# kei312/stereoanywhere

Hardware: AMD Instinct MI355X
Metric: stereo pairs/sec @540x960 D=192 (1/2/4/8 GPU) + EPE vs reference (higher is better)
Workload: dtype f32 (F(4x4) Winograd-domain and direct-conv products as exact f16 hi/lo pair products on MFMA, fp32 accumulation; everything else fp32); 1 GPU; configs[1]: batch 4/GPU x 540x960 (padded 544x960), 22 GRU iters, published flags; global_batch=4, iters=22, parallelism=dp1 (independent pairs, metrics all_gather)

## Files before the change

stereoanywhere_amd/csrc/conv2d_wino4.hip:

```cpp
#include "sa_common.h"

#include <algorithm>
#include <cstdlib>
#include <type_traits>

#pragma clang fp contract(fast)

namespace {

using sa::f32x4, sa::f32x2, sa::f16x2, sa::f16x4;

constexpr int NPT = 36;

template <int NW_, int KC_, bool SPLIT_ = false>
struct W4Cfg {
  static constexpr bool SPLIT = SPLIT_;
  static constexpr int NW = NW_, NTHR = 64 * NW_, TG = NW_ / 2, NT = 16 * TG, KC = KC_, JPC = KC_ / 4;
  static constexpr int NR = 6;
  static constexpr int CO = 32, CG = 2;
  static constexpr int SB = 4 * CO;
  static constexpr int PS_MAX = NT == 64 ? 340 : 204;
  static constexpr int PBUF = (KC * PS_MAX + 63) / 64 * 64 * 4;
  static constexpr int UBUF = NPT * KC * CO;
  static constexpr int BUF = PBUF + UBUF;
// ... 526 lines not shown
    __syncthreads();
  }
#pragma unroll 1
  for (int kc = 0; kc < nchunks; ++kc) {
    const int cur = kc & 1;
    if constexpr (AFF) {
      asm volatile("s_waitcnt vmcnt(0)" ::: "memory");
      float *pbuf = smem + cur * BUF;
#pragma unroll
      for (int j = 0; j < PDMA; ++j) {
        const int pcj = (int)((pcs >> (4 * j)) & 15u) - 1;
        if (pcj >= 0) {
          f32x4 *q = reinterpret_cast<f32x4 *>(pbuf + ((wv + NWAVE * j) * 64 + lane) * 4);
          const float2 ab = atab[kc * KC + pcj];
          f32x4 v = *q;
#pragma unroll
          for (int e = 0; e < 4; ++e) v[e] = fmaxf(v[e] * ab.x + ab.y, act_floor);
          *q = v;
        }
      }
    }
    if constexpr (SPLIT && !AFF) {
      if (scaled) {
        asm volatile("s_waitcnt vmcnt(0)" ::: "memory");
        float *pbuf = smem + cur * BUF + (wv * 64 + lane) * 4;
#pragma unroll 1
        for (int j = 0; j < PDMA; ++j) {
          if (wv + NWAVE * j < npi) {
            f32x4 *q = reinterpret_cast<f32x4 *>(pbuf + NWAVE * j * 256);
            *q = *q * xscale;
          }
        }
      }
    }
    __syncthreads();
    const float *pb = smem + cur * BUF + pread;
    const float *ub = smem + cur * BUF + PBUF + uread;
    f32x2 ra[6], rc[6];
    f32x4 rb[6];
    auto load_rows = [&](int s, int r0, int r1) __attribute__((always_inline)) {
      const float *p = pb + s * 4 * PSv * 4;
#pragma unroll
      for (int r = r0; r < r1; ++r) {
        ra[r] = *reinterpret_cast<const f32x2 *>(p + r * PGv * 4);
        rb[r] = *reinterpret_cast<const f32x4 *>(p + r * PGv * 4 + 2);
        rc[r] = *reinterpret_cast<const f32x2 *>(p + r * PGv * 4 + 6);
      }
    };
    f32xg bc[NR], bn[NR];
    auto load_b = [&](int s, int jj, f32xg *b) __attribute__((always_inline)) {
#pragma unroll
      for (int i = 0; i < NR; ++i) {
        if constexpr (SPLIT) {
          const float *q = ub + (6 * i + 3 * HF + jj) * JPC * SB + s;
          b[i] = f32xg{q[0], q[JPC]};
        } else {
          b[i] = *reinterpret_cast<const f32xg *>(ub + ((6 * i + 3 * HF + jj) * JPC + s) * SB);
        }
      }
    };
    if constexpr (W4Paired<C, AFF>) {
      float t0[6][3], t1[6][3];
      load_rows(0, 0, 6);
#pragma unroll
      for (int r = 0; r < 6; ++r) bt6h<HF>(ra[r].y, rb[r].x, rb[r].y, rb[r].z, rb[r].w, rc[r].x, t0[r]);
      load_rows(1, 0, 6);
#pragma unroll
      for (int r = 0; r < 6; ++r) bt6h<HF>(ra[r].y, rb[r].x, rb[r].y, rb[r].z, rb[r].w, rc[r].x, t1[r]);
      f32x4 pc_[NR];
      auto load_bp = [&](int jj, int i0, int i1, f32x4 (&b)[NR]) __attribute__((always_inline)) {
#pragma unroll
        for (int i = i0; i < i1; ++i) b[i] = *reinterpret_cast<const f32x4 *>(ub + (6 * i + 3 * HF + jj) * JPC * SB);
      };
#pragma unroll
      for (int jj = 0; jj < 3; ++jj) {
        if (kc + 1 < nchunks) {
          issue_part(kc + 1, cur ^ 1, jj);
          __builtin_amdgcn_sched_barrier(0);
        }
        load_bp(jj, 0, NR / 2, pc_);
        float v0[6], v1[6];
        bt6(t0[0][jj], t0[1][jj], t0[2][jj], t0[3][jj], t0[4][jj], t0[5][jj], v0);
        bt6(t1[0][jj], t1[1][jj], t1[2][jj], t1[3][jj], t1[4][jj], t1[5][jj], v1);
#pragma unroll
        for (int i = 0; i < NR; ++i) {
          if (i == 1) load_bp(jj, NR / 2, NR, pc_);
          if constexpr (HALF) {
            const f16x4 ahi = w4_pair_half(v0[i], v1[i]);
#pragma unroll
            for (int g = 0; g < CG; ++g) {
              const f16x4 bp = __builtin_bit_cast(f16x4, g == 0 ? pc_[i].xy : pc_[i].zw);
              acc[i][jj][g] = __builtin_amdgcn_mfma_f32_16x16x16f16(ahi, bp, acc[i][jj][g], 0, 0, 0);
            }
          } else {
            f16x4 ahi, alo;
            w4_pair_split(v0[i], v1[i], ahi, alo);
#pragma unroll
            for (int g = 0; g < CG; ++g) {
              const f16x4 bp = __builtin_bit_cast(f16x4, g == 0 ? pc_[i].xy : pc_[i].zw);
              acc[i][jj][g] = __builtin_amdgcn_mfma_f32_16x16x16f16(ahi, bp, acc[i][jj][g], 0, 0, 0);
              acc[i][jj][g] = __builtin_amdgcn_mfma_f32_16x16x16f16(alo, bp, acc[i][jj][g], 0, 0, 0);
            }
          }
        }
        __builtin_amdgcn_sched_barrier(0);
      }
    } else {
      load_rows(0, 0, 6);
      load_b(0, 0, bc);
#pragma unroll
      for (int s = 0; s < JPC; ++s) {
        if (s == 1) load_rows(1, 3, 6);
        float t[6][3];
#pragma unroll
        for (int r = 0; r < 6; ++r) bt6h<HF>(ra[r].y, rb[r].x, rb[r].y, rb[r].z, rb[r].w, rc[r].x, t[r]);
        if (s + 1 < JPC) load_rows(1, 0, 3);
#pragma unroll
        for (int jj = 0; jj < 3; ++jj) {
          if (s == 0 && kc + 1 < nchunks) {
            issue_part(kc + 1, cur ^ 1, jj);
            __builtin_amdgcn_sched_barrier(0);
          }
          if (s + 1 < JPC || jj < 2) load_b(jj < 2 ? s : s + 1, jj < 2 ? jj + 1 : 0, bn);
          float v[6];
          bt6(t[0][jj], t[1][jj], t[2][jj], t[3][jj], t[4][jj], t[5][jj], v);
          if constexpr (SPLIT) {
            static_assert(HALF, "an unpaired split config is the half config");
#pragma unroll
            for (int i = 0; i < NR; ++i) {
              const f16x4 a = __builtin_shufflevector(__builtin_convertvector(f32x2{v[i], v[i]}, f16x2),
                                                      f16x2{(_Float16)0.0f, (_Float16)0.0f}, 0, 1, 2, 3);
              const f16x4 b0 = __builtin_bit_cast(f16x4, f32x2{bc[i][0], bc[i][0]});
              const f16x4 b1 = __builtin_bit_cast(f16x4, f32x2{bc[i][1], bc[i][1]});
              acc[i][jj][0] = __builtin_amdgcn_mfma_f32_16x16x16f16(a, b0, acc[i][jj][0], 0, 0, 0);
              acc[i][jj][1] = __builtin_amdgcn_mfma_f32_16x16x16f16(a, b1, acc[i][jj][1], 0, 0, 0);
            }
          } else {
#pragma unroll
            for (int i = 0; i < NR; ++i)
#pragma unroll
              for (int g = 0; g < CG; ++g)
                acc[i][jj][g] = __builtin_amdgcn_mfma_f32_16x16x4f32(v[i], bc[i][g],
                                                                      acc[i][jj][g], 0, 0, 0);
          }
          __builtin_amdgcn_sched_barrier(0);

#pragma unroll
          for (int i = 0; i < NR; ++i) bc[i] = bn[i];
        }
      }
    }
  }
  __syncthreads();
  if constexpr (SPLIT) {
    const float inv_scale = 1.0f / ((float)(1 << W4S_LOG2) * xscale);
#pragma unroll
    for (int i = 0; i < NR; ++i)
#pragma unroll
      for (int jj = 0; jj < 3; ++jj)
#pragma unroll
        for (int g = 0; g < CG; ++g) acc[i][jj][g] *= inv_scale;
  }

  float *ot = smem;
  const int relu = P.relu;
  f32x4 chk = f32x4{0.f, 0.f, 0.f, 0.f};
  float whead = 0.0f;
  if constexpr (GATED && C::NTHR == 512)
    if (gate->mode == 3 && tid < C::CO * 9) whead = gate->head_w[co0 * 9 + tid];
#pragma unroll
  for (int phase = 0; phase < 2; ++phase) {
#pragma unroll
  for (int gi = 0; gi < CG / 2; ++gi) {
    const int g = 2 * gi + (phase == 0 ? 1 - HF : HF);
    const int col = g * 16 + (lane & 15);
    const float bv = phase == 1 ? bpre[gi] : 0.0f;
#pragma unroll
    for (int i = 0; i < 4; ++i) {
      const int ti = tg * 16 + w4_tile_of_row(4 * (lane >> 4) + i), orow = (ti >> ltw) * 4, ocol = (ti & (tw - 1)) * 4;
      float u[4][3];
#pragma unroll
      for (int jj = 0; jj < 3; ++jj) {
        float mcol[6], o[4];
#pragma unroll
        for (int a = 0; a < 6; ++a) mcol[a] = acc[a][jj][g][i];
        at6(mcol, o);
#pragma unroll
        for (int a = 0; a < 4; ++a) u[a][jj] = o[a];
      }
#pragma unroll
      for (int a = 0; a < 4; ++a) {
        const f32x4 y = at6h<HF>(u[a][0], u[a][1], u[a][2]);
        f32x4 *o = reinterpret_cast<f32x4 *>(ot + col * OPP + (orow + a) * BW + ocol);
        if (phase == 0) {
          *o = y;
        } else {
          f32x4 v = (HF == 0 ? (*o + y) : (y + *o)) + bv;
          if constexpr (SPLIT) chk += v;
          if (relu) v = f32x4{fmaxf(v.x, 0.0f), fmaxf(v.y, 0.0f), fmaxf(v.z, 0.0f), fmaxf(v.w, 0.0f)};
          *o = v;
        }
      }
    }
  }
    if (phase == 0) __syncthreads();
  }
  if constexpr (SPLIT) {
    static_assert(C::CO * C::OPP + C::CO * 9 + NWAVE <= C::SMEM, "range guard flags");
    int *flags = reinterpret_cast<int *>(smem + C::CO * C::OPP + C::CO * 9);
    const float t = (chk.x + chk.y) + (chk.z + chk.w);
    const bool wbad = __builtin_amdgcn_ballot_w64(!__builtin_isfinite(t)) != 0;
    if (lane == 0) flags[wv] = wbad ? 1 : 0;
    __syncthreads();
    int any = 0;
#pragma unroll
    for (int w = 0; w < NWAVE; ++w) any |= flags[w];
    if (any && guard) return true;
  } else {
    __syncthreads();
  }
  if constexpr (GATED && C::NTHR == 512) {
    if (gate->mode == 3) {
      w4_flowhead<C, LTW>(P, *gate, smem, n, co0, st, y0, x0, tid, whead);
      return false;
    }
  }
  w4_emit<C, GATED, C::CO>(P, gate, ot, 0, n, co0, st, tiles_w, y0, x0, BH, BW, ltw + 2, tid);
  return false;
}

template <class C, bool GATED, bool AFF = false>
__global__ __launch_bounds__(C::NTHR, C::NW == 8 ? 1 : 2) void wino_f4k3_kernel(const W4Launch L) {
  const unsigned g = blockIdx.x;
  int pi = 0;
#pragma unroll
  for (int i = 1; i < MAX_PROB; ++i) pi += (i < L.nprob && g >= L.end[i - 1]) ? 1 : 0;
  const unsigned base = pi ? L.end[pi - 1] : 0u, nb = L.nblk[pi];
  if (g - base >= nb) return;
  __shared__ __attribute__((aligned(16))) float smem[C::SMEM];
  __shared__ float2 atab[AFF ? C::AFF_MAX : 1];
  const unsigned wid = sa::xcd_remap(g - base, nb);
  const bool guard = C::SPLIT && L.guard;
  const W4Prob &P = L.p[pi];
  const W4Gate *gp = GATED ? &L.gate[pi] : nullptr;
  bool over;
#define W4_BODY(CC_, HF_, LTW_, G_, XS_) w4_body<CC_, HF_, LTW_, GATED, AFF>(P, gp, wid, smem, atab, G_, XS_)
  if (threadIdx.x < C::NTHR / 2) over = P.ltw == 4 ? W4_BODY(C, 0, 4, guard, 1.0f) : W4_BODY(C, 0, 5, guard, 1.0f);
  else over = P.ltw == 4 ? W4_BODY(C, 1, 4, guard, 1.0f) : W4_BODY(C, 1, 5, guard, 1.0f);
  if constexpr (C::SPLIT) {
    if (over) {
      __syncthreads();
      if (threadIdx.x == 0) atomicAdd(&g_w4_redo_blocks, 1u);
      int pil = __builtin_amdgcn_readfirstlane(pi);
      unsigned widl = __builtin_amdgcn_readfirstlane(wid);
      asm volatile("" : "+s"(pil), "+s"(widl));
      const W4Prob &P2 = L.p[pil];
      const W4Gate *gp2 = GATED ? &L.gate[pil] : nullptr;
#define W4_BODY2(HF_, LTW_) w4_body<C, HF_, LTW_, GATED, AFF>(P2, gp2, widl, smem, atab, false, 0.0f)
      if (threadIdx.x < C::NTHR / 2) {
        if (P2.ltw == 4) W4_BODY2(0, 4);
        else W4_BODY2(0, 5);
      } else {
        if (P2.ltw == 4) W4_BODY2(1, 4);
        else W4_BODY2(1, 5);
      }
#undef W4_BODY2
    }
  }
#undef W4_BODY
}

__global__ __launch_bounds__(256) void wino4_weights_kernel(const float *__restrict__ w, int Cout, int Cin, int CB,
                                                            float *__restrict__ U) {
  const long i = (long)blockIdx.x * blockDim.x + threadIdx.x;
  if (i >= (long)Cout * Cin) return;
  const int co = (int)(i / Cin), ci = (int)(i % Cin);
  const float *g = w + i * 9;
  const double G[6][3] = {{0.25, 0.0, 0.0},
                          {-1.0 / 6, -1.0 / 6, -1.0 / 6},
                          {-1.0 / 6, 1.0 / 6, -1.0 / 6},
                          {1.0 / 24, 1.0 / 12, 1.0 / 6},
                          {1.0 / 24, -1.0 / 12, 1.0 / 6},
                          {0.0, 0.0, 1.0}};
  double t[6][3];
  for (int a = 0; a < 6; ++a)
    for (int c = 0; c < 3; ++c) t[a][c] = G[a][0] * g[c] + G[a][1] * g[3 + c] + G[a][2] * g[6 + c];
  const int chunk = ci / 8, s = (ci % 8) / 4, k = ci % 4, cb = co / CB, c = co % CB, ng = CB / 16;
  for (int a = 0; a < 6; ++a)
    for (int b = 0; b < 6; ++b) {
      const double u = t[a][0] * G[b][0] + t[a][1] * G[b][1] + t[a][2] * G[b][2];
      const int pt = 6 * a + b;
      U[(((((long)cb * (Cin / 8) + chunk) * NPT + pt) * 2 + s) * 4 + k) * CB + (c & 15) * ng + (c >> 4)] = (float)u;
    }
}

__global__ __launch_bounds__(256) void wino4s_weights_kernel(const float *__restrict__ w, int Cout, int Cin,
                                                             unsigned *__restrict__ U) {
  const long i = (long)blockIdx.x * blockDim.x + threadIdx.x;
  if (i >= (long)Cout * Cin) return;
  const int co = (int)(i / Cin), ci = (int)(i % Cin);
  const float *g = w + i * 9;
  const double G[6][3] = {{0.25, 0.0, 0.0},
                          {-1.0 / 6, -1.0 / 6, -1.0 / 6},
                          {-1.0 / 6, 1.0 / 6, -1.0 / 6},
                          {1.0 / 24, 1.0 / 12, 1.0 / 6},
                          {1.0 / 24, -1.0 / 12, 1.0 / 6},
                          {0.0, 0.0, 1.0}};
  double t[6][3];
  for (int a = 0; a < 6; ++a)
    for (int c = 0; c < 3; ++c) t[a][c] = G[a][0] * g[c] + G[a][1] * g[3 + c] + G[a][2] * g[6 + c];
  const int chunk = ci / 8, s = (ci % 8) / 4, k = ci % 4, cb = co / 32, gg = (co % 32) / 16, n = co % 16;
  for (int a = 0; a < 6; ++a)
    for (int b = 0; b < 6; ++b) {
      const double u = (t[a][0] * G[b][0] + t[a][1] * G[b][1] + t[a][2] * G[b][2]) * (double)(1 << W4S_LOG2);
      const _Float16 hi = (_Float16)(float)u;
      const _Float16 lo = (_Float16)(float)(u - (double)hi);
      const unsigned pr = (unsigned)__builtin_bit_cast(unsigned short, hi) |
                          ((unsigned)__builtin_bit_cast(unsigned short, lo) << 16);
      const int pt = 6 * a + b;
      U[((((((long)cb * (Cin / 8) + chunk) * NPT + pt) * 4 + k) * 16 + n) * 2 + gg) * 2 + s] = pr;
    }
}


__global__ __launch_bounds__(256) void flow_head_reduce_kernel(const float *__restrict__ part, long part_bs, int ncb,
                                                               int H, int W, int BH, int BW, int tiles_w,
                                                               int tiles_hw, const float *__restrict__ bias0,
                                                               float *__restrict__ cx, float *__restrict__ fa,
                                                               long fa_bs, float *__restrict__ fb, long fb_bs) {
  const unsigned r = blockIdx.x * 256u + threadIdx.x;
  const unsigned hw = (unsigned)(H * W);
  if (r >= hw) return;
  const long b = blockIdx.y;
  const int y = (int)(r / (unsigned)W), x = (int)(r % (unsigned)W);
  const int RH = BH + 2, RW = BW + 2, tiles_h = tiles_hw / tiles_w;
  const int ty0 = y / BH, tx0 = x / BW;
  const bool up = y % BH == 0 && ty0 > 0, dn = y % BH == BH - 1 && ty0 + 1 < tiles_h;
  const bool lf = x % BW == 0 && tx0 > 0, rt = x % BW == BW - 1 && tx0 + 1 < tiles_w;
  const int ty1 = up ? ty0 - 1 : ty0 + 1, tx1 = lf ? tx0 - 1 : tx0 + 1;
  auto off = [&](int ty, int tx) { return ((long)(ty * tiles_w + tx) * RH + (y - (ty * BH - 1))) * RW + (x - (tx * BW - 1)); };
  const bool hy = up || dn, hx = lf || rt;
  const long o0 = off(ty0, tx0), o1 = hx ? off(ty0, tx1) : o0, o2 = hy ? off(ty1, tx0) : o0,
             o3 = hx && hy ? off(ty1, tx1) : o0;
  float d = bias0[0];
  const float *pc = part + b * part_bs;
  const long cbs = (long)tiles_hw * RH * RW;
  for (int cb0 = 0; cb0 < ncb; cb0 += 8) {
    float a[8][4];
#pragma unroll
    for (int j = 0; j < 8; ++j) {
// ... 219 lines not shown
```

stereoanywhere_amd/csrc/conv_direct.hip:

```cpp
#include "sa_common.h"

#pragma clang fp contract(fast)

namespace {

using sa::f32x4, sa::f32x2, sa::f16x2, sa::f16x4;

constexpr float DSP_SCALE = 4096.0f;
__device__ __forceinline__ f16x4 dsplit(const float x) {
  const f16x2 hh = __builtin_convertvector(f32x2{x, x}, f16x2);
  float l;
  asm("v_fma_mix_f32 %0, -%1, 1.0, %2 op_sel_hi:[1,0,0]" : "=v"(l) : "v"(__builtin_bit_cast(unsigned, hh)), "v"(x));
  const f16x2 ll = __builtin_convertvector(f32x2{l, l}, f16x2);
  return __builtin_shufflevector(hh, ll, 0, 1, 2, 3);
}

__device__ __forceinline__ float dunsplit(const float packed) {
  const f16x2 p = __builtin_bit_cast(f16x2, packed);
  return (float)p[0] + (float)p[1];
}

__device__ unsigned g_direct_redo_blocks;

constexpr int DOTH = 8, DOTW = 32, MT = 2;

template <int K, int S, int KC, int NTL, bool DS>
struct DCfg {
  static constexpr int PH = (DOTH - 1) * S + K, PW = (DOTW - 1) * S + K;
  static constexpr int PWP = PW;
  static constexpr int PL0 = PH * PWP, PR = S == 1 ? 16 : 17;
  static constexpr int PLANE = PL0 + ((PR - PL0 % 32) + 32) % 32;
  static constexpr int XN = KC * PLANE;
  static constexpr int NC = 16 * NTL;
  static constexpr int KK = K * K;
  static constexpr int WN = KC * KK * NC;
  static constexpr int DN = DS ? KC * NC : 0;
  static constexpr int NCP = NC + 16;
  static constexpr int WROWS = KC * KK + (DS ? KC : 0);
  static constexpr int XPT = (XN + 511) / 512, WPT = (WN + DN) / 4 / 512 + (((WN + DN) / 4) % 512 ? 1 : 0);
  static constexpr int KSTEPS = KC * KK / 4;
  static constexpr int NACC = NTL * (DS ? 2 : 1);
  static constexpr int SMEM = XN + WROWS * NCP + 4;
  static_assert(KC % 4 == 0, "a K-step of 4 must stay inside one tap");
  static_assert((WN + DN) % 4 == 0, "weights are staged as float4");
  static_assert(SMEM * 4 <= 160 * 1024, "LDS budget");
  static_assert(8 * 2 * NACC * 16 * 2 <= SMEM, "the stats reduction reuses the staging LDS");
};

struct DirArgs {
  const float *in;
  long in_bs;
  const float *skip, *cm, *cs;
  long skip_bs;
  int Cin, H, W, Ho, Wo;
  const float *wg, *wd;
  int Cout, co_blocks, tiles_w, tiles, nchunks;
  float *out, *out_ds;
  long out_bs, out_ds_bs;
  double *part, *part_ds;
};

__device__ __forceinline__ float close_value(float v, float m, float s, float k) {
#pragma clang fp contract(off)
  const float y = fmaxf((v - m) * s + 0.0f, 0.0f);
  return fmaxf(y + k, 0.0f);
}

template <int K, int S, int KC, int NTL, bool DS, bool SP = false, bool CL = false>
__global__ __launch_bounds__(512, DS ? 2 : 4) void conv_direct_kernel(const DirArgs a) {
  using C = DCfg<K, S, KC, NTL, DS>;
  constexpr int NC = C::NC, NCP = C::NCP, PLANE = C::PLANE, PWP = C::PWP;
  __shared__ __attribute__((aligned(16))) float sm[C::SMEM];
  __shared__ float ctab[CL ? 2 : 1][CL ? 2 * KC : 1];
  float *sx = sm, *sw = sm + C::XN, *sd = sw + KC * C::KK * NCP;
  constexpr int SPARE = C::SMEM - 4;
  const int tid = threadIdx.x, lane = tid & 63;
  const int wv = __builtin_amdgcn_readfirstlane(tid >> 6);
  const unsigned wid = sa::xcd_remap(blockIdx.x, gridDim.x);
  const int cb = wid % a.co_blocks;
  const int st = (wid / a.co_blocks) % a.tiles;
  const int n = wid / (a.co_blocks * a.tiles);
  const int oy0 = (st / a.tiles_w) * DOTH, ox0 = (st % a.tiles_w) * DOTW;
  const int iy0 = oy0 * S - K / 2, ix0 = ox0 * S - K / 2;
  const long hw = (long)a.H * a.W;
  const float *src = a.in + (long)n * a.in_bs;

  constexpr int OOB = 0x7ffffff0;
  const __amdgpu_buffer_rsrc_t xin = __builtin_amdgcn_make_buffer_rsrc(
      const_cast<float *>(src), (short)0, (int)((long)a.Cin * hw * 4), 0x00020000);
  int xoff[C::XPT], xl[C::XPT];
#pragma unroll
  for (int j = 0; j < C::XPT; ++j) {
    const int i = tid + 512 * j;
    const int ci = i / PLANE, rem = i % PLANE, r = rem / PWP, c = rem % PWP;
    const int y = iy0 + r, x = ix0 + c;
    const bool ok = i < C::XN && rem < C::PH * PWP && c < C::PW && y >= 0 && y < a.H && x >= 0 && x < a.W;
    xoff[j] = ok ? (int)((min(ci, a.Cin - 1) * hw + (long)y * a.W + x) * 4) : OOB;
    xl[j] = i < C::XN ? i : SPARE;
  }
  constexpr int WQ = (C::WN + C::DN) / 4;
  const __amdgpu_buffer_rsrc_t win = __builtin_amdgcn_make_buffer_rsrc(
      const_cast<float *>(a.wg) + (long)cb * a.nchunks * C::WN, (short)0, (int)((long)a.nchunks * C::WN * 4),
      0x00020000);
  const __amdgpu_buffer_rsrc_t din = __builtin_amdgcn_make_buffer_rsrc(
      const_cast<float *>(DS ? a.wd + (long)cb * a.nchunks * C::DN : a.wg), (short)0,
      (int)((long)a.nchunks * (DS ? C::DN : 0) * 4), 0x00020000);
  int woff[C::WPT], wl[C::WPT];
  bool wds[C::WPT];
#pragma unroll
  for (int j = 0; j < C::WPT; ++j) {
    const int i = tid + 512 * j;
    wds[j] = i >= C::WN / 4;
    woff[j] = i < WQ ? (wds[j] ? (i - C::WN / 4) * 16 : i * 16) : OOB;
    const int row = (4 * i) / NC, col = (4 * i) % NC;
    wl[j] = i < WQ ? row * NCP + col : SPARE;
  }
  const __amdgpu_buffer_rsrc_t kin = __builtin_amdgcn_make_buffer_rsrc(
      const_cast<float *>(CL ? a.skip + (long)n * a.skip_bs : src), (short)0, (int)((long)a.Cin * hw * 4), 0x00020000);
  float xr[C::XPT], kr[CL ? C::XPT : 1];
  float tv = 0.0f;
  f32x4 wr[C::WPT];
  auto fetch = [&](int chunk) __attribute__((always_inline)) {
    const int xs = chunk * KC * (int)hw * 4;
#pragma unroll
    for (int j = 0; j < C::XPT; ++j) xr[j] = __uint_as_float(__builtin_amdgcn_raw_buffer_load_b32(xin, xoff[j], xs, 0));
    if constexpr (CL) {
#pragma unroll
      for (int j = 0; j < C::XPT; ++j) kr[j] = __uint_as_float(__builtin_amdgcn_raw_buffer_load_b32(kin, xoff[j], xs, 0));
      if (tid < 2 * KC) {
        const int c = min(chunk * KC + tid % KC, a.Cin - 1);
        tv = (tid < KC ? a.cm : a.cs)[(long)n * a.Cin + c];
      }
    }
#pragma unroll
    for (int j = 0; j < C::WPT; ++j) {
      const auto v = wds[j] ? __builtin_amdgcn_raw_buffer_load_b128(din, woff[j], chunk * C::DN * 4, 0)
                            : __builtin_amdgcn_raw_buffer_load_b128(win, woff[j], chunk * C::WN * 4, 0);
      wr[j] = f32x4{__uint_as_float(v[0]), __uint_as_float(v[1]), __uint_as_float(v[2]), __uint_as_float(v[3])};
    }
  };
  auto put_tab = [&](int chunk) __attribute__((always_inline)) {
    if (CL && tid < 2 * KC) ctab[CL ? chunk & 1 : 0][tid] = tv;
  };
  auto commit = [&](int chunk) __attribute__((always_inline)) {
#pragma unroll
    for (int j = 0; j < C::XPT; ++j) {
      float v = xr[j];
      if constexpr (CL) {
        const int cl = min((tid + 512 * j) / PLANE, KC - 1);
        const float *tb = ctab[chunk & 1];
        v = xoff[j] == OOB ? 0.0f : close_value(v, tb[cl], tb[KC + cl], kr[j]);
      }
      sx[xl[j]] = v;
    }
#pragma unroll
    for (int j = 0; j < C::WPT; ++j) *reinterpret_cast<f32x4 *>(sw + wl[j]) = wr[j];
  };

  f32x4 acc[MT][C::NACC];
#pragma unroll
  for (int m = 0; m < MT; ++m)
#pragma unroll
    for (int t = 0; t < C::NACC; ++t) acc[m][t] = f32x4{0.f, 0.f, 0.f, 0.f};
  const int kq = lane >> 4, ml = lane & 15;
  int abase[MT];
#pragma unroll
  for (int m = 0; m < MT; ++m) abase[m] = kq * PLANE + (wv * S) * PWP + (m * 16 + ml) * S;
  const int bbase = kq * NCP + ml;

  fetch(0);
  if constexpr (CL) {
    put_tab(0);
    __syncthreads();
  }
  commit(0);
  __syncthreads();
#pragma unroll 1
  for (int chunk = 0; chunk < a.nchunks; ++chunk) {
    if (chunk + 1 < a.nchunks) fetch(chunk + 1);
#pragma unroll
    for (int s = 0; s < C::KSTEPS; ++s) {
      const int tap = (4 * s) / KC, ci0 = (4 * s) % KC;
      const int koff = ci0 * PLANE + (tap / K) * PWP + (tap % K);
      float av[MT];
#pragma unroll
      for (int m = 0; m < MT; ++m) av[m] = sx[abase[m] + koff];
      auto prod = [&](const float bv, f32x4 *ac) __attribute__((always_inline)) {
        if constexpr (SP) {
          const f16x4 b = __builtin_bit_cast(f16x4, f32x2{bv, bv});
#pragma unroll
          for (int m = 0; m < MT; ++m) ac[m * C::NACC] = __builtin_amdgcn_mfma_f32_16x16x16f16(dsplit(av[m]), b, ac[m * C::NACC], 0, 0, 0);
        } else {
#pragma unroll
          for (int m = 0; m < MT; ++m) ac[m * C::NACC] = __builtin_amdgcn_mfma_f32_16x16x4f32(av[m], bv, ac[m * C::NACC], 0, 0, 0);
        }
      };
#pragma unroll
      for (int t = 0; t < NTL; ++t) prod(sw[bbase + 4 * s * NCP + t * 16], &acc[0][t]);
      if (DS && tap == (K / 2) * K + K / 2) {
#pragma unroll
        for (int t = 0; t < NTL; ++t) prod(sd[bbase + ci0 * NCP + t * 16], &acc[0][NTL + t]);
      }
    }
    if (CL && chunk + 1 < a.nchunks) put_tab(chunk + 1);
    __syncthreads();
    if (chunk + 1 < a.nchunks) {
      commit(chunk + 1);
      __syncthreads();
    }
  }
  if constexpr (SP) {
    f32x4 sum = f32x4{0.f, 0.f, 0.f, 0.f};
#pragma unroll
    for (int m = 0; m < MT; ++m)
#pragma unroll
      for (int t = 0; t < C::NACC; ++t) sum += acc[m][t];
    const float tot = (sum.x + sum.y) + (sum.z + sum.w);
    if (__syncthreads_or(!__builtin_isfinite(tot))) {
      if (tid == 0) atomicAdd(&g_direct_redo_blocks, 1u);
#pragma unroll
      for (int m = 0; m < MT; ++m)
#pragma unroll
        for (int t = 0; t < C::NACC; ++t) acc[m][t] = f32x4{0.f, 0.f, 0.f, 0.f};
#pragma unroll 1
      for (int chunk = 0; chunk < a.nchunks; ++chunk) {
        fetch(chunk);
        if constexpr (CL) {
          put_tab(chunk);
          __syncthreads();
        }
        commit(chunk);
        __syncthreads();
#pragma unroll 1
        for (int s = 0; s < C::KSTEPS; ++s) {
          const int tap = (4 * s) / KC, ci0 = (4 * s) % KC;
          const int koff = ci0 * PLANE + (tap / K) * PWP + (tap % K);
#pragma unroll
          for (int t = 0; t < NTL; ++t) {
            const float w = dunsplit(sw[bbase + 4 * s * NCP + t * 16]);
#pragma unroll
            for (int m = 0; m < MT; ++m)
              acc[m][t] = __builtin_amdgcn_mfma_f32_16x16x4f32(sx[abase[m] + koff], w, acc[m][t], 0, 0, 0);
          }
          if (DS && tap == (K / 2) * K + K / 2) {
#pragma unroll
            for (int t = 0; t < NTL; ++t) {
              const float w = dunsplit(sd[bbase + ci0 * NCP + t * 16]);
#pragma unroll
              for (int m = 0; m < MT; ++m)
                acc[m][NTL + t] = __builtin_amdgcn_mfma_f32_16x16x4f32(sx[abase[m] + koff], w, acc[m][NTL + t], 0, 0, 0);
            }
          }
        }
        __syncthreads();
      }
    }
  }

  if constexpr (SP) {
#pragma unroll
    for (int m = 0; m < MT; ++m)
#pragma unroll
      for (int t = 0; t < C::NACC; ++t) acc[m][t] *= 1.0f / DSP_SCALE;
  }
  double *red = reinterpret_cast<double *>(sm);
  constexpr int RC = C::NACC * 16;
  const int oy = oy0 + wv;
  const bool stats = a.part != nullptr;
  const bool interior = oy0 + DOTH <= a.Ho && ox0 + DOTW <= a.Wo && (a.Wo & 3) == 0;
#pragma unroll
  for (int t = 0; t < C::NACC; ++t) {
    const bool ds = DS && t >= NTL;
    const int co = cb * NC + (ds ? t - NTL : t) * 16 + ml;
    float *dst = (ds ? a.out_ds + (long)n * a.out_ds_bs : a.out + (long)n * a.out_bs) + (long)co * a.Ho * a.Wo;
    double s1 = 0.0, s2 = 0.0;
    if (interior) {
#pragma unroll
      for (int m = 0; m < MT; ++m) {
        const int ox = ox0 + m * 16 + 4 * kq;
        *reinterpret_cast<float4 *>(dst + (long)oy * a.Wo + ox) =
            make_float4(acc[m][t][0], acc[m][t][1], acc[m][t][2], acc[m][t][3]);
#pragma unroll
        for (int r = 0; r < 4; ++r) {
          const double v = acc[m][t][r];
          s1 += v;
          s2 += v * v;
        }
      }
    } else {
#pragma unroll
      for (int m = 0; m < MT; ++m) {
        const int ox = ox0 + m * 16 + 4 * kq;
#pragma unroll
        for (int r = 0; r < 4; ++r) {
          if (oy < a.Ho && ox + r < a.Wo) {
            const float v = acc[m][t][r];
            dst[(long)oy * a.Wo + ox + r] = v;
            s1 += (double)v;
            s2 += (double)v * v;
          }
        }
      }
    }
    if (stats) {
      s1 += __shfl_xor(s1, 16);
      s2 += __shfl_xor(s2, 16);
      s1 += __shfl_xor(s1, 32);
      s2 += __shfl_xor(s2, 32);
      if (kq == 0) {
        red[(wv * 2 + 0) * RC + t * 16 + ml] = s1;
        red[(wv * 2 + 1) * RC + t * 16 + ml] = s2;
      }
    }
  }
  if (stats) {
    __syncthreads();
    for (int c = tid; c < RC; c += 512) {
      double s1 = 0.0, s2 = 0.0;
#pragma unroll
      for (int w = 0; w < 8; ++w) {
        s1 += red[(w * 2 + 0) * RC + c];
        s2 += red[(w * 2 + 1) * RC + c];
      }
      const bool ds = DS && c >= NC;
      double *pp = ds ? a.part_ds : a.part;
      if (pp) {
        const int co = cb * NC + (ds ? c - NC : c);
        pp += (((long)n * a.Cout + co) * a.tiles + st) * 2;
        pp[0] = s1;
        pp[1] = s2;
      }
    }
  }
}

__global__ void direct_weights_kernel(const float *__restrict__ w, int Cout, int Cin, int K, int KC, int NC,
                                      int nchunks, int ds, float *__restrict__ out) {
  const long total = (long)Cout * nchunks * KC * K * K;
  const long i = (long)blockIdx.x * blockDim.x + threadIdx.x;
  if (i >= total) return;
  const int n = (int)(i % NC);
  long r = i / NC;
  const int ci = (int)(r % KC);
  r /= KC;
  const int tap = (int)(r % (K * K));
  r /= K * K;
  const int chunk = (int)(r % nchunks);
  const int cblk = (int)(r / nchunks);
  const int co = cblk * NC + n, cin = chunk * KC + ci;
  (void)ds;
  out[i] = cin < Cin ? w[((long)co * Cin + cin) * K * K + tap] : 0.0f;
}

bool pick(int K, int S, int Cout, int &KC, int &NTL) {
  KC = K == 7 ? 4 : 8;
  if (K == 7 && S == 1 && Cout % 64 == 0) { NTL = 4; return true; }
  if ((K == 3 || K == 1) && S == 2 && Cout == 96) { NTL = 6; return true; }
  if ((K == 3 || K == 1) && S == 2 && Cout % 128 == 0) { NTL = 8; return true; }
  return false;
}

}

extern "C" int sa_conv_direct_weights(const float *weight, int Cout, int Cin, int K, int S, int with_ds,
                                      float *out, void *stream) {
  int KC = 0, NTL = 0;
  SA_REQUIRE(weight && out && Cout > 0 && Cin > 0, "sa_conv_direct_weights: bad arguments");
  SA_REQUIRE(pick(K, S, Cout, KC, NTL) && (K != 1 || with_ds), "sa_conv_direct_weights: no kernel for K=%d S=%d Cout=%d",
             K, S, Cout);
  const int NC = 16 * NTL, nchunks = (Cin + KC - 1) / KC;
  const long total = (long)Cout * nchunks * KC * K * K;
  hipStream_t s = sa::as_stream(stream);
  direct_weights_kernel<<<(unsigned)((total + 255) / 256), 256, 0, s>>>(weight, Cout, Cin, K, KC, NC, nchunks, 0,
                                                                       out);
  return sa::check_launch("sa_conv_direct_weights");
}

namespace {
__global__ void direct_split_kernel(const float *__restrict__ w, long n, unsigned *__restrict__ out) {
  const long i = (long)blockIdx.x * blockDim.x + threadIdx.x;
  if (i >= n) return;
  const double u = (double)w[i] * DSP_SCALE;
  const _Float16 hi = (_Float16)(float)u;
  const _Float16 lo = (_Float16)(float)(u - (double)hi);
  out[i] = (unsigned)__builtin_bit_cast(unsigned short, hi) | ((unsigned)__builtin_bit_cast(unsigned short, lo) << 16);
}

}

extern "C" int sa_conv_direct_weights_split(const float *arranged, long n, void *out, void *stream) {
  SA_REQUIRE(arranged && out && n > 0, "sa_conv_direct_weights_split: bad arguments");
  hipStream_t s = sa::as_stream(stream);
  direct_split_kernel<<<(unsigned)((n + 255) / 256), 256, 0, s>>>(arranged, n, static_cast<unsigned *>(out));
  return sa::check_launch("sa_conv_direct_weights_split");
}

long sa_direct_redo_blocks_internal(int reset) {
  return sa::read_redo_counter(g_direct_redo_blocks, reset, false);
}

extern "C" long sa_conv_direct_weights_size(int Cout, int Cin, int K, int S, int with_ds) {
  int KC = 0, NTL = 0;
  if (!pick(K, S, Cout, KC, NTL) || (K == 1 && !with_ds)) return -1;
  return (long)Cout * ((Cin + KC - 1) / KC) * KC * K * K;
}

extern "C" long sa_conv_direct_stat_parts(int Ho, int Wo) {
  return (long)((Wo + DOTW - 1) / DOTW) * ((Ho + DOTH - 1) / DOTH);
}

template <bool SP>
static int conv_direct_launch(const float *in, long in_bs, int N, int Cin, int H, int W, int K, int S,
                              const float *wg, const float *wd, int Cout, float *out, long out_bs, float *out_ds,
                              long out_ds_bs, double *part, double *part_ds, void *stream,
                              const float *skip = nullptr, long skip_bs = 0, const float *cm = nullptr,
                              const float *cs = nullptr) {
  int KC = 0, NTL = 0;
  const bool ds = wd != nullptr, cl = skip != nullptr;
  SA_REQUIRE(in && wg && out && N > 0 && Cin > 0 && H > 0 && W > 0, "sa_conv_direct: bad arguments");
  SA_REQUIRE(!ds || out_ds, "sa_conv_direct: downsample weights without an output");
  SA_REQUIRE(K != 1 && pick(K, S, Cout, KC, NTL) && ds == (S == 2),
             "sa_conv_direct: no kernel for K=%d S=%d Cout=%d ds=%d", K, S, Cout, (int)ds);
  SA_REQUIRE((long)Cin * H * W < (1L << 31), "sa_conv_direct: image too large");
  SA_REQUIRE(Cin % KC == 0 || Cin <= KC, "sa_conv_direct: Cin must be a multiple of %d (or at most %d)", KC, KC);
  SA_REQUIRE(!cl || (cm && cs && K == 3 && Cin % KC == 0),
             "sa_conv_direct_close: needs mean / rstd, a 3x3 stride-2 conv and Cin %% %d == 0", KC);
  const int p = K / 2;
  const int Ho = (H + 2 * p - K) / S + 1, Wo = (W + 2 * p - K) / S + 1;
  const int tiles_w = (Wo + DOTW - 1) / DOTW, tiles = tiles_w * ((Ho + DOTH - 1) / DOTH);
  const int co_blocks = Cout / (16 * NTL);
  const DirArgs a{in, in_bs, skip, cm, cs, skip_bs, Cin, H, W, Ho, Wo, wg, wd, Cout, co_blocks, tiles_w, tiles,
                  (Cin + KC - 1) / KC, out, out_ds, out_bs, out_ds_bs, part, part_ds};
  const long nblk = (long)N * tiles * co_blocks;
  SA_REQUIRE(nblk < (1L << 31), "sa_conv_direct: grid too large");
  hipStream_t s = sa::as_stream(stream);
  sa::TimingScope ts(SA_K_CONV_DIRECT, s);
  if (K == 7) {
    conv_direct_kernel<7, 1, 4, 4, false, SP><<<(unsigned)nblk, 512, 0, s>>>(a);
  } else if (NTL == 6) {
    if (cl) conv_direct_kernel<3, 2, 8, 6, true, SP, true><<<(unsigned)nblk, 512, 0, s>>>(a);
    else conv_direct_kernel<3, 2, 8, 6, true, SP><<<(unsigned)nblk, 512, 0, s>>>(a);
  } else {
    SA_REQUIRE(!cl, "sa_conv_direct_close: no close form for Cout = %d", Cout);
    conv_direct_kernel<3, 2, 8, 8, true, SP><<<(unsigned)nblk, 512, 0, s>>>(a);
  }
  return sa::check_launch("sa_conv_direct");
}

extern "C" int sa_conv_direct(const float *in, long in_bs, int N, int Cin, int H, int W, int K, int S,
                              const float *wg, const float *wd, int Cout, float *out, long out_bs, float *out_ds,
                              long out_ds_bs, double *part, double *part_ds, void *stream) {
  return conv_direct_launch<false>(in, in_bs, N, Cin, H, W, K, S, wg, wd, Cout, out, out_bs, out_ds, out_ds_bs, part,
                                   part_ds, stream);
}

extern "C" int sa_conv_direct_split(const float *in, long in_bs, int N, int Cin, int H, int W, int K, int S,
                                    const void *wg, const void *wd, int Cout, float *out, long out_bs, float *out_ds,
                                    long out_ds_bs, double *part, double *part_ds, void *stream) {
  return conv_direct_launch<true>(in, in_bs, N, Cin, H, W, K, S, static_cast<const float *>(wg),
                                  static_cast<const float *>(wd), Cout, out, out_bs, out_ds, out_ds_bs, part, part_ds,
                                  stream);
}

extern "C" int sa_conv_direct_close_supported(int K, int S, int Cout) {
  int KC = 0, NTL = 0;
  return K == 3 && S == 2 && pick(K, S, Cout, KC, NTL) && NTL == 6 ? 1 : 0;
}

extern "C" int sa_conv_direct_close(const float *c2, long c2_bs, const float *skip, long skip_bs, const float *mean,
                                    const float *rstd, int N, int Cin, int H, int W, int K, int S, const void *wg,
                                    const void *wd, int split, int Cout, float *out, long out_bs, float *out_ds,
                                    long out_ds_bs, double *part, double *part_ds, void *stream) {
  SA_REQUIRE(skip, "sa_conv_direct_close: null skip");
  if (split)
    return conv_direct_launch<true>(c2, c2_bs, N, Cin, H, W, K, S, static_cast<const float *>(wg),
                                    static_cast<const float *>(wd), Cout, out, out_bs, out_ds, out_ds_bs, part, part_ds,
                                    stream, skip, skip_bs, mean, rstd);
  return conv_direct_launch<false>(c2, c2_bs, N, Cin, H, W, K, S, static_cast<const float *>(wg),
                                   static_cast<const float *>(wd), Cout, out, out_bs, out_ds, out_ds_bs, part, part_ds,
                                   stream, skip, skip_bs, mean, rstd);
}
```

Measured before the change: 69.76 pairs/s.

## Pack split-f16 direct-conv operands for 16x16x32 MFMA and fold Winograd rescale into bias

In the split-precision direct conv, weights are pre-split into f16 hi/lo fragments laid out in LDS by tap step. Activations are split eight at a time, so each product runs as three 16x16x32 f16 MFMAs (hi*hi, hi*lo, lo*hi) instead of many 16x16x16 MFMAs with a duplicated operand. The 7x7 stem is limited to a single channel chunk. Separately, the Winograd split path drops the per-accumulator rescale loop and applies the scale with an FMA alongside the bias in the epilogue. This adds a new fragment-staging scheme, more LDS use, and a dropped lo*lo term that the old path may have partly covered.

Measured after the change: 69.95 pairs/s (median of 6 runs). No clear change (+0.3%).

```diff
diff --git a/stereoanywhere_amd/csrc/conv2d_wino4.hip b/stereoanywhere_amd/csrc/conv2d_wino4.hip
--- a/stereoanywhere_amd/csrc/conv2d_wino4.hip
+++ b/stereoanywhere_amd/csrc/conv2d_wino4.hip
@@ -702,15 +702,7 @@
     }
   }
   __syncthreads();
-  if constexpr (SPLIT) {
-    const float inv_scale = 1.0f / ((float)(1 << W4S_LOG2) * xscale);
-#pragma unroll
-    for (int i = 0; i < NR; ++i)
-#pragma unroll
-      for (int jj = 0; jj < 3; ++jj)
-#pragma unroll
-        for (int g = 0; g < CG; ++g) acc[i][jj][g] *= inv_scale;
-  }
+  const float inv_scale = SPLIT ? 1.0f / ((float)(1 << W4S_LOG2) * xscale) : 1.0f;
 
   float *ot = smem;
   const int relu = P.relu;
@@ -745,7 +737,13 @@
         if (phase == 0) {
           *o = y;
         } else {
-          f32x4 v = (HF == 0 ? (*o + y) : (y + *o)) + bv;
+          f32x4 v = HF == 0 ? (*o + y) : (y + *o);
+          if constexpr (SPLIT) {
+            v = f32x4{__builtin_fmaf(v.x, inv_scale, bv), __builtin_fmaf(v.y, inv_scale, bv),
+                      __builtin_fmaf(v.z, inv_scale, bv), __builtin_fmaf(v.w, inv_scale, bv)};
+          } else {
+            v = v + bv;
+          }
           if constexpr (SPLIT) chk += v;
           if (relu) v = f32x4{fmaxf(v.x, 0.0f), fmaxf(v.y, 0.0f), fmaxf(v.z, 0.0f), fmaxf(v.w, 0.0f)};
           *o = v;
diff --git a/stereoanywhere_amd/csrc/conv_direct.hip b/stereoanywhere_amd/csrc/conv_direct.hip
--- a/stereoanywhere_amd/csrc/conv_direct.hip
+++ b/stereoanywhere_amd/csrc/conv_direct.hip
@@ -4,20 +4,26 @@
 
 namespace {
 
-using sa::f32x4, sa::f32x2, sa::f16x2, sa::f16x4;
+using sa::f32x4, sa::f32x2, sa::f16x2, sa::f16x8;
+using u32x4 = __attribute__((ext_vector_type(4))) unsigned;
+using u32x2 = __attribute__((ext_vector_type(2))) unsigned;
 
 constexpr float DSP_SCALE = 4096.0f;
-__device__ __forceinline__ f16x4 dsplit(const float x) {
-  const f16x2 hh = __builtin_convertvector(f32x2{x, x}, f16x2);
-  float l;
-  asm("v_fma_mix_f32 %0, -%1, 1.0, %2 op_sel_hi:[1,0,0]" : "=v"(l) : "v"(__builtin_bit_cast(unsigned, hh)), "v"(x));
-  const f16x2 ll = __builtin_convertvector(f32x2{l, l}, f16x2);
-  return __builtin_shufflevector(hh, ll, 0, 1, 2, 3);
-}
-
-__device__ __forceinline__ float dunsplit(const float packed) {
-  const f16x2 p = __builtin_bit_cast(f16x2, packed);
-  return (float)p[0] + (float)p[1];
+__device__ __forceinline__ void dsplit8(const float (&x)[8], f16x8 &ahi, f16x8 &alo) {
+  f16x2 h[4], q[4];
+#pragma unroll
+  for (int p = 0; p < 4; ++p) {
+    h[p] = __builtin_convertvector(f32x2{x[2 * p], x[2 * p + 1]}, f16x2);
+    float l0, l1;
+    asm("v_fma_mix_f32 %0, -%1, 1.0, %2 op_sel_hi:[1,0,0]" : "=v"(l0) : "v"(__builtin_bit_cast(unsigned, h[p])), "v"(x[2 * p]));
+    asm("v_fma_mix_f32 %0, -%1, 1.0, %2 op_sel:[1,0,0] op_sel_hi:[1,0,0]"
+        : "=v"(l1) : "v"(__builtin_bit_cast(unsigned, h[p])), "v"(x[2 * p + 1]));
+    q[p] = __builtin_convertvector(f32x2{l0, l1}, f16x2);
+  }
+  ahi = __builtin_shufflevector(__builtin_shufflevector(h[0], h[1], 0, 1, 2, 3),
+                                __builtin_shufflevector(h[2], h[3], 0, 1, 2, 3), 0, 1, 2, 3, 4, 5, 6, 7);
+  alo = __builtin_shufflevector(__builtin_shufflevector(q[0], q[1], 0, 1, 2, 3),
+                                __builtin_shufflevector(q[2], q[3], 0, 1, 2, 3), 0, 1, 2, 3, 4, 5, 6, 7);
 }
 
 __device__ unsigned g_direct_redo_blocks;
@@ -41,6 +47,18 @@
   static constexpr int KSTEPS = KC * KK / 4;
   static constexpr int NACC = NTL * (DS ? 2 : 1);
   static constexpr int SMEM = XN + WROWS * NCP + 4;
+  static constexpr int CPL = KC / 4, TPS = 8 / CPL;
+  static constexpr int STEPS = (KK + TPS - 1) / TPS;
+  static constexpr int CT = (K / 2) * K + K / 2;
+  static constexpr int NF = STEPS + (DS ? 1 : 0);
+  static constexpr int FRAG = NTL * 512;
+  static constexpr int PJ = NTL * 64 * 2 <= 512 ? 4 : 8;
+  static constexpr int UPF = NTL * 64 * (8 / PJ);
+  static constexpr int SMEM_SP = XN + NF * FRAG + 4;
+  static_assert(KC == 4 || KC == 8, "a lane holds 1 or 2 channels of a tap");
+  static_assert(!DS || CT % TPS == 0, "the 1x1 takes the first slot of the centre tap's step");
+  static_assert(UPF <= 512 && PJ % CPL == 0 && XN % 4 == 0, "fragment staging");
+  static_assert(SMEM_SP * 4 <= 160 * 1024, "LDS budget");
   static_assert(KC % 4 == 0, "a K-step of 4 must stay inside one tap");
   static_assert((WN + DN) % 4 == 0, "weights are staged as float4");
   static_assert(SMEM * 4 <= 160 * 1024, "LDS budget");
@@ -70,10 +88,11 @@
 __global__ __launch_bounds__(512, DS ? 2 : 4) void conv_direct_kernel(const DirArgs a) {
   using C = DCfg<K, S, KC, NTL, DS>;
   constexpr int NC = C::NC, NCP = C::NCP, PLANE = C::PLANE, PWP = C::PWP;
-  __shared__ __attribute__((aligned(16))) float sm[C::SMEM];
+  constexpr int SMEM = SP ? C::SMEM_SP : C::SMEM;
+  __shared__ __attribute__((aligned(16))) float sm[SMEM];
   __shared__ float ctab[CL ? 2 : 1][CL ? 2 * KC : 1];
   float *sx = sm, *sw = sm + C::XN, *sd = sw + KC * C::KK * NCP;
-  constexpr int SPARE = C::SMEM - 4;
+  constexpr int SPARE = SMEM - 4;
   const int tid = threadIdx.x, lane = tid & 63;
   const int wv = __builtin_amdgcn_readfirstlane(tid >> 6);
   const unsigned wid = sa::xcd_remap(blockIdx.x, gridDim.x);
@@ -105,10 +124,11 @@
   const __amdgpu_buffer_rsrc_t din = __builtin_amdgcn_make_buffer_rsrc(
       const_cast<float *>(DS ? a.wd + (long)cb * a.nchunks * C::DN : a.wg), (short)0,
       (int)((long)a.nchunks * (DS ? C::DN : 0) * 4), 0x00020000);
-  int woff[C::WPT], wl[C::WPT];
-  bool wds[C::WPT];
-#pragma unroll
-  for (int j = 0; j < C::WPT; ++j) {
+  constexpr int WPT = SP ? 0 : C::WPT;
+  int woff[WPT ? WPT : 1], wl[WPT ? WPT : 1];
+  bool wds[WPT ? WPT : 1];
+#pragma unroll
+  for (int j = 0; j < WPT; ++j) {
     const int i = tid + 512 * j;
     wds[j] = i >= C::WN / 4;
     woff[j] = i < WQ ? (wds[j] ? (i - C::WN / 4) * 16 : i * 16) : OOB;
@@ -119,7 +139,12 @@
       const_cast<float *>(CL ? a.skip + (long)n * a.skip_bs : src), (short)0, (int)((long)a.Cin * hw * 4), 0x00020000);
   float xr[C::XPT], kr[CL ? C::XPT : 1];
   float tv = 0.0f;
-  f32x4 wr[C::WPT];
+  f32x4 wr[WPT ? WPT : 1];
+  const int whq = tid / (4 * NC), wkg = (tid / NC) % 4, wc = tid % NC;
+  const bool wact = C::UPF == 512 || tid < C::UPF;
+  const int wbo = ((whq * (C::PJ / C::CPL) * KC + wkg) * NC + wc) * 4;
+  const int wdst = (wc / 16) * 512 + (wkg * 16 + wc % 16) * 4 + whq * (C::PJ / 2);
+  unsigned wq[SP ? C::NF : 1][SP ? C::PJ : 1];
   auto fetch = [&](int chunk) __attribute__((always_inline)) {
     const int xs = chunk * KC * (int)hw * 4;
 #pragma unroll
@@ -132,8 +157,28 @@
         tv = (tid < KC ? a.cm : a.cs)[(long)n * a.Cin + c];
       }
     }
-#pragma unroll
-    for (int j = 0; j < C::WPT; ++j) {
+    if constexpr (SP) {
+      if (wact) {
+#pragma unroll
+        for (int f = 0; f < C::NF; ++f)
+#pragma unroll
+          for (int jj = 0; jj < C::PJ; ++jj) {
+            const bool isds = DS && f == C::STEPS;
+            const int tap = f * C::TPS + jj / C::CPL;
+            if (isds ? jj >= C::CPL : tap >= C::KK) {
+              wq[f][jj] = 0u;
+              continue;
+            }
+            const int imm = ((isds ? 0 : tap * KC) + 4 * (jj % C::CPL)) * NC * 4;
+            const bool tail = C::PJ < 8 && f * C::TPS + (C::PJ + jj) / C::CPL >= C::KK;
+            const int off = (tail && whq != 0 ? OOB : wbo) + imm;
+            wq[f][jj] = isds ? __builtin_amdgcn_raw_buffer_load_b32(din, off, chunk * C::DN * 4, 0)
+                             : __builtin_amdgcn_raw_buffer_load_b32(win, off, chunk * C::WN * 4, 0);
+          }
+      }
+    }
+#pragma unroll
+    for (int j = 0; j < WPT; ++j) {
       const auto v = wds[j] ? __builtin_amdgcn_raw_buffer_load_b128(din, woff[j], chunk * C::DN * 4, 0)
                             : __builtin_amdgcn_raw_buffer_load_b128(win, woff[j], chunk * C::WN * 4, 0);
       wr[j] = f32x4{__uint_as_float(v[0]), __uint_as_float(v[1]), __uint_as_float(v[2]), __uint_as_float(v[3])};
@@ -154,7 +199,28 @@
       sx[xl[j]] = v;
     }
 #pragma unroll
-    for (int j = 0; j < C::WPT; ++j) *reinterpret_cast<f32x4 *>(sw + wl[j]) = wr[j];
+    for (int j = 0; j < WPT; ++j) *reinterpret_cast<f32x4 *>(sw + wl[j]) = wr[j];
+    if constexpr (SP) {
+      if (wact) {
+#pragma unroll
+        for (int f = 0; f < C::NF; ++f) {
+          unsigned hi[C::PJ / 2], lo[C::PJ / 2];
+#pragma unroll
+          for (int p = 0; p < C::PJ / 2; ++p) {
+            hi[p] = __builtin_amdgcn_perm(wq[f][2 * p + 1], wq[f][2 * p], 0x05040100u);
+            lo[p] = __builtin_amdgcn_perm(wq[f][2 * p + 1], wq[f][2 * p], 0x07060302u);
+          }
+          float *d = sw + f * C::FRAG + wdst;
+          if constexpr (C::PJ == 8) {
+            *reinterpret_cast<u32x4 *>(d) = u32x4{hi[0], hi[1], hi[2], hi[3]};
+            *reinterpret_cast<u32x4 *>(d + 256) = u32x4{lo[0], lo[1], lo[2], lo[3]};
+          } else {
+            *reinterpret_cast<u32x2 *>(d) = u32x2{hi[0], hi[1]};
+            *reinterpret_cast<u32x2 *>(d + 256) = u32x2{lo[0], lo[1]};
+          }
+        }
+      }
+    }
   };
 
   f32x4 acc[MT][C::NACC];
@@ -168,6 +234,7 @@
   for (int m = 0; m < MT; ++m) abase[m] = kq * PLANE + (wv * S) * PWP + (m * 16 + ml) * S;
   const int bbase = kq * NCP + ml;
 
+  const int nchunks = SP && K == 7 ? 1 : a.nchunks;
   fetch(0);
   if constexpr (CL) {
     put_tab(0);
@@ -176,35 +243,63 @@
   commit(0);
   __syncthreads();
 #pragma unroll 1
-  for (int chunk = 0; chunk < a.nchunks; ++chunk) {
-    if (chunk + 1 < a.nchunks) fetch(chunk + 1);
-#pragma unroll
-    for (int s = 0; s < C::KSTEPS; ++s) {
-      const int tap = (4 * s) / KC, ci0 = (4 * s) % KC;
-      const int koff = ci0 * PLANE + (tap / K) * PWP + (tap % K);
-      float av[MT];
-#pragma unroll
-      for (int m = 0; m < MT; ++m) av[m] = sx[abase[m] + koff];
-      auto prod = [&](const float bv, f32x4 *ac) __attribute__((always_inline)) {
-        if constexpr (SP) {
-          const f16x4 b = __builtin_bit_cast(f16x4, f32x2{bv, bv});
-#pragma unroll
-          for (int m = 0; m < MT; ++m) ac[m * C::NACC] = __builtin_amdgcn_mfma_f32_16x16x16f16(dsplit(av[m]), b, ac[m * C::NACC], 0, 0, 0);
-        } else {
+  for (int chunk = 0; chunk < nchunks; ++chunk) {
+    if (chunk + 1 < nchunks) fetch(chunk + 1);
+    if constexpr (SP) {
+#pragma unroll
+      for (int s = 0; s < C::STEPS; ++s) {
+        f16x8 ahi[MT], alo[MT];
+#pragma unroll
+        for (int m = 0; m < MT; ++m) {
+          float v[8];
+#pragma unroll
+          for (int j = 0; j < 8; ++j) {
+            const int tap = s * C::TPS + j / C::CPL;
+            v[j] = tap < C::KK ? sx[abase[m] + (j % C::CPL) * 4 * PLANE + (tap / K) * PWP + (tap % K)] : 0.0f;
+          }
+          dsplit8(v, ahi[m], alo[m]);
+        }
+        auto prod = [&](const int f, f32x4 *ac) __attribute__((always_inline)) {
+#pragma unroll
+          for (int t = 0; t < NTL; ++t) {
+            const float *b = sw + f * C::FRAG + t * 512 + lane * 4;
+            const f16x8 bhi = *reinterpret_cast<const f16x8 *>(b), blo = *reinterpret_cast<const f16x8 *>(b + 256);
+#pragma unroll
+            for (int m = 0; m < MT; ++m) {
+              f32x4 c = ac[m * C::NACC + t];
+              c = __builtin_amdgcn_mfma_f32_16x16x32_f16(ahi[m], bhi, c, 0, 0, 0);
+              c = __builtin_amdgcn_mfma_f32_16x16x32_f16(ahi[m], blo, c, 0, 0, 0);
+              c = __builtin_amdgcn_mfma_f32_16x16x32_f16(alo[m], bhi, c, 0, 0, 0);
+              ac[m * C::NACC + t] = c;
+            }
+          }
+        };
+        prod(s, &acc[0][0]);
+        if (DS && s == C::CT / C::TPS) prod(C::STEPS, &acc[0][NTL]);
+      }
+    } else {
+#pragma unroll
+      for (int s = 0; s < C::KSTEPS; ++s) {
+        const int tap = (4 * s) / KC, ci0 = (4 * s) % KC;
+        const int koff = ci0 * PLANE + (tap / K) * PWP + (tap % K);
+        float av[MT];
+#pragma unroll
+        for (int m = 0; m < MT; ++m) av[m] = sx[abase[m] + koff];
+        auto prod = [&](const float bv, f32x4 *ac) __attribute__((always_inline)) {
 #pragma unroll
           for (int m = 0; m < MT; ++m) ac[m * C::NACC] = __builtin_amdgcn_mfma_f32_16x16x4f32(av[m], bv, ac[m * C::NACC], 0, 0, 0);
-        }
-      };
-#pragma unroll
-      for (int t = 0; t < NTL; ++t) prod(sw[bbase + 4 * s * NCP + t * 16], &acc[0][t]);
-      if (DS && tap == (K / 2) * K + K / 2) {
-#pragma unroll
-        for (int t = 0; t < NTL; ++t) prod(sd[bbase + ci0 * NCP + t * 16], &acc[0][NTL + t]);
-      }
-    }
-    if (CL && chunk + 1 < a.nchunks) put_tab(chunk + 1);
+        };
+#pragma unroll
+        for (int t = 0; t < NTL; ++t) prod(sw[bbase + 4 * s * NCP + t * 16], &acc[0][t]);
+        if (DS && tap == (K / 2) * K + K / 2) {
+#pragma unroll
+          for (int t = 0; t < NTL; ++t) prod(sd[bbase + ci0 * NCP + t * 16], &acc[0][NTL + t]);
+        }
+      }
+    }
+    if (CL && chunk + 1 < nchunks) put_tab(chunk + 1);
     __syncthreads();
-    if (chunk + 1 < a.nchunks) {
+    if (chunk + 1 < nchunks) {
       commit(chunk + 1);
       __syncthreads();
     }
@@ -222,8 +317,13 @@
       for (int m = 0; m < MT; ++m)
 #pragma unroll
         for (int t = 0; t < C::NACC; ++t) acc[m][t] = f32x4{0.f, 0.f, 0.f, 0.f};
+      const _Float16 *swh = reinterpret_cast<const _Float16 *>(sw) + lane * 8;
+      auto weight = [&](int f, int t, int slot) __attribute__((always_inline)) {
+        const _Float16 *q = swh + (f * C::FRAG + t * 512) * 2 + slot;
+        return (float)q[0] + (float)q[512];
+      };
 #pragma unroll 1
-      for (int chunk = 0; chunk < a.nchunks; ++chunk) {
+      for (int chunk = 0; chunk < nchunks; ++chunk) {
         fetch(chunk);
         if constexpr (CL) {
           put_tab(chunk);
@@ -237,7 +337,7 @@
           const int koff = ci0 * PLANE + (tap / K) * PWP + (tap % K);
 #pragma unroll
           for (int t = 0; t < NTL; ++t) {
-            const float w = dunsplit(sw[bbase + 4 * s * NCP + t * 16]);
+            const float w = weight(tap / C::TPS, t, (tap % C::TPS) * C::CPL + ci0 / 4);
 #pragma unroll
             for (int m = 0; m < MT; ++m)
               acc[m][t] = __builtin_amdgcn_mfma_f32_16x16x4f32(sx[abase[m] + koff], w, acc[m][t], 0, 0, 0);
@@ -245,7 +345,7 @@
           if (DS && tap == (K / 2) * K + K / 2) {
 #pragma unroll
             for (int t = 0; t < NTL; ++t) {
-              const float w = dunsplit(sd[bbase + ci0 * NCP + t * 16]);
+              const float w = weight(C::STEPS, t, ci0 / 4);
 #pragma unroll
               for (int m = 0; m < MT; ++m)
                 acc[m][NTL + t] = __builtin_amdgcn_mfma_f32_16x16x4f32(sx[abase[m] + koff], w, acc[m][NTL + t], 0, 0, 0);
@@ -423,6 +523,7 @@
              "sa_conv_direct: no kernel for K=%d S=%d Cout=%d ds=%d", K, S, Cout, (int)ds);
   SA_REQUIRE((long)Cin * H * W < (1L << 31), "sa_conv_direct: image too large");
   SA_REQUIRE(Cin % KC == 0 || Cin <= KC, "sa_conv_direct: Cin must be a multiple of %d (or at most %d)", KC, KC);
+  SA_REQUIRE(!(SP && K == 7) || Cin <= KC, "sa_conv_direct_split: the 7x7 stem takes Cin <= %d", KC);
   SA_REQUIRE(!cl || (cm && cs && K == 3 && Cin % KC == 0),
              "sa_conv_direct_close: needs mean / rstd, a 3x3 stride-2 conv and Cin %% %d == 0", KC);
   const int p = K / 2;
```
